# jkxing/EPSM_Mitsuba3

Hardware: AMD Instinct MI355X
Metric: manifold_paths_per_s (higher is better)
Workload: dtype f32

## Files before the change

### __graft_entry__.py

```python
from __future__ import annotations

import os
import subprocess
import sys

ROOT = os.path.dirname(os.path.abspath(__file__))
if ROOT not in sys.path:
    sys.path.insert(0, ROOT)


def build() -> None:
    env = dict(os.environ)
    targets = [("epsm_mitsuba3_amd/csrc", "epsm_mitsuba3_amd/libepsm_hip.so"),
               ("oracle", "oracle/libepsm_oracle.so"),
               ("examples", "examples/build/epsm_host_driver"),
               ("tests/host_harness", "tests/host_harness/libtrace_host.so")]
    for d, out in targets:
        path = os.path.join(ROOT, out)
        before = os.path.getmtime(path) if os.path.isfile(path) else None
        subprocess.run(["make", "-C", os.path.join(ROOT, d), "-s"], check=True, env=env)
        after = os.path.getmtime(path)
        print(f"build_mode {out}: {'up-to-date' if before == after else 'compiled'}", flush=True)
    for script, out in (("_forward_host.py", "tests/host_harness/libtrace_fwd_host.so"),
                        ("_texture_host.py", "tests/host_harness/libtrace_tex_host.so"),
                        ("_bsdf_host.py", "tests/host_harness/libtrace_bsdf_host.so"),
                        ("_material_host.py", "tests/host_harness/libtrace_material_host.so"),
                        ("_alphamap_host.py", "tests/host_harness/libtrace_alphamap_host.so")):
        path = os.path.join(ROOT, out)
        before = os.path.getmtime(path) if os.path.isfile(path) else None
        subprocess.run([sys.executable, "-B", os.path.join(ROOT, "tests", script)], check=True,
                       env=dict(env, PYTHONPATH=ROOT + os.pathsep + env.get("PYTHONPATH", "")))
        after = os.path.getmtime(path) if os.path.isfile(path) else None
        print(f"build_mode {out}: {'up-to-date' if before == after else 'compiled'}", flush=True)
    import epsm_mitsuba3_amd
    from epsm_mitsuba3_amd import _lib
    lib = _lib.lib()
    assert lib.epsm_abi_version() == _lib.ABI_VERSION == 7


def smoke() -> None:
    import torch
    import epsm_mitsuba3_amd as epsm
    from epsm_mitsuba3_amd.synth import synth_path_info, path_info_to
    from oracle.binding import oracle_calc_grad

    assert torch.cuda.is_available(), "smoke() needs cuda:0"
# ... 58 lines not shown
```

### epsm_mitsuba3_amd/_lib.py

```python
from __future__ import annotations

import ctypes as C
import os
import subprocess

import torch

_HERE = os.path.dirname(os.path.abspath(__file__))
ABI_VERSION = 7
LIB_PATH = os.path.join(_HERE, os.environ.get("EPSM_LIB_NAME", "libepsm_hip.so"))
_lib = None


class EpsmError(RuntimeError):
    pass


class build_lock:

    def __init__(self, directory: str):
        self.path = os.path.join(directory, ".build.lock")

    @staticmethod
    def _open(path: str):
# ... 202 lines not shown
    global _lib
    if _lib is None:
        if not os.path.isfile(LIB_PATH):
            raise EpsmError(
                f"{LIB_PATH} not found: build it with `python -c 'import __graft_entry__ as g; g.build()'` "
                "(or make -C epsm_mitsuba3_amd/csrc). There is no CPU fallback.")
        _lib = _declare(C.CDLL(LIB_PATH))
        if _lib.epsm_abi_version() != ABI_VERSION:
            raise EpsmError("libepsm_hip.so ABI version mismatch")
    return _lib


def stream(device):
    device = torch.device(device)
    return torch.cuda.current_stream(device).cuda_stream if device.type == "cuda" else None


def check(rc: int, what: str):
    if rc != 0:
        msg = lib().epsm_last_error().decode("utf-8", "replace")
        raise EpsmError(f"{what} failed with code {rc}: {msg}")


OPT_SMALL_WAVEFRONT_PATHS, OPT_REPLICAS, OPT_ONE_LAUNCH = 0, 1, 2


class options:

    def __init__(self, small_wavefront_paths=None, replicas=None, one_launch=None):
        self.want = {OPT_SMALL_WAVEFRONT_PATHS: small_wavefront_paths, OPT_REPLICAS: None if replicas is None else int(bool(replicas)),
                     OPT_ONE_LAUNCH: None if one_launch is None else int(bool(one_launch))}

    def __enter__(self):
        self.saved = {k: lib().epsm_get_option(k) for k, v in self.want.items() if v is not None}
        for k, v in self.want.items():
            if v is not None:
                check(lib().epsm_set_option(k, int(v)), "epsm_set_option")
        return self

    def __exit__(self, *exc):
        for k, v in self.saved.items():
            lib().epsm_set_option(k, v)
        return False
```

### epsm_mitsuba3_amd/csrc/epsm_backward_cp.hip

```cpp
#include <stdlib.h>
#include <string.h>

#define EPSM_FAST_RCP64
#include "epsm_fused.h"
#include "epsm_cp_core.h"
#include "epsm_wave_scatter.h"

using namespace epsm;

namespace {

#ifndef EPSM_CP_THREADS
#define EPSM_CP_THREADS 256
#endif
#ifndef EPSM_CP_OCC
#define EPSM_CP_OCC 3
#endif
#ifndef EPSM_CP_ROWS_FLOAT
#define EPSM_CP_ROWS_FLOAT 2064
#endif
#ifndef EPSM_CP_ROWS_FIXED
#define EPSM_CP_ROWS_FIXED 1184
#endif
#ifndef EPSM_CP_QUEUE
#define EPSM_CP_QUEUE 192
#endif
#ifndef EPSM_CP_BLOCKS
#define EPSM_CP_BLOCKS (1 << 20)
#endif
constexpr int kThreads = EPSM_CP_THREADS, kWaves = kThreads / 64, kQueueCap = EPSM_CP_QUEUE;
constexpr int kKeys = 6;
constexpr int kStashFirstItem = 64;
static_assert(kQueueCap - kStashFirstItem >= 128, "the stash needs 128 queue items");

__device__ __forceinline__ int div_small(int lane, int c) {
    const int inv = c == 1 ? 65536 : c == 2 ? 32768 : c == 3 ? 21846 : c == 4 ? 16384 : 13108;
    return (lane * inv) >> 16;
}

__device__ __forceinline__ int up1_bits(int v) { return __builtin_amdgcn_update_dpp(v, v, 0x138, 0xf, 0xf, false); }
__device__ __forceinline__ int down1_bits(int v) { return __builtin_amdgcn_update_dpp(v, v, 0x130, 0xf, 0xf, false); }
__device__ __forceinline__ float up1(float v) { return __int_as_float(up1_bits(__float_as_int(v))); }
__device__ __forceinline__ float down1(float v) { return __int_as_float(down1_bits(__float_as_int(v))); }
__device__ __forceinline__ int up1(int v) { return up1_bits(v); }
__device__ __forceinline__ int down1(int v) { return down1_bits(v); }
// ... 114 lines not shown
        }
        {
            gm = fin(gm);
            bool v = on && nz3(gm) && bid < (uint64_t) F.B;
            if (__ballot(v) != 0ull) {
                V3<float> val[1] = {mk3<float>(v ? dot(gm, dhf) : 0.f, 0.f, 0.f)};
                const uint32_t aid[3] = {2u * (uint32_t) F.V + bid, 0u, 0u};
                push<1>(v, aid, val);
            }
        }
        {
            gdiff = fin(gdiff);
            const bool v = live && nz3(gdiff) && tri_ok(tn, F.V) && (tn.w & kModePos);
            group(v, gdiff, nb0, nb1, tn.x, tn.y, tn.z);
        }
        {
            const float dis = bits_to_float(sh.w);
            const bool v = d1 && nz3(dpf) && tri_ok(ts, F.V) && (ts.w & kModePos) && dis != 0.f;
            group(v, dpf * dis, bits_to_float(sh.y), bits_to_float(sh.z), ts.x, ts.y, ts.z);
        }
    }
};

struct LaneId { int q, c, k; uint32_t plan; int loc; };
struct Rounds {
    int cls[kKeys + 1], rb[kKeys + 1];
    const uint16_t *perm;
    const uint32_t *plan;
    __device__ __forceinline__ LaneId lane_of(int r, int lane) const {
        LaneId L;
        int q = 0;
#pragma unroll
        for (int t = 1; t < kKeys; ++t) if (r >= rb[t]) q = t;
        int cls_q = cls[0], n_q = cls[1] - cls[0], rb_q = rb[0], ppr = 64;
#pragma unroll
        for (int t = 1; t < kKeys; ++t) if (q == t) { cls_q = cls[t]; n_q = cls[t + 1] - cls[t]; rb_q = rb[t]; ppr = 64 / t; }
        const int c = q > 0 ? q : 1;
        const int j = div_small(lane, c), k = lane - j * c + 1;
        const int idx = (r - rb_q) * ppr + j;
        const bool lane_on = r >= 0 && r < rb[kKeys] && j < ppr && idx < n_q;
        const int loc = lane_on ? (int) perm[cls_q + idx] : 0;
        L.q = q; L.c = c; L.k = k; L.loc = loc;
        L.plan = lane_on ? plan[loc] : 0u;
        return L;
    }
};

typedef float F2v __attribute__((ext_vector_type(2)));
typedef float F3v __attribute__((ext_vector_type(3)));
struct GeoFetch {
    F4v o0, o1, o2, o3, o4, o5;
    float o_lz;
    F4v p0, p1, p2;
    F4v n0, n1, n2;
    float gx, gy;
};
struct AddrFetch {
    F4v q6;
    F4v q7;
    U4 sh;
};
__device__ __forceinline__ F2v ld2(const float *p) { return *(const __attribute__((address_space(1))) F2v *) p; }
struct WinBase {
    const float *verts, *rays;
    const float *sub_rec;
    int64_t sub_path;
// ... 15 lines not shown
        B.sub_path = (p >= 0 && p < F.g.N) ? p : 0;
        B.sub_rec = F.pk_verts + B.sub_path * F.pk_path_stride;
    }
    B.rays = F.pk_rays + base * F.pk_ray_stride;
    B.shadow = F.pk_shadow ? F.pk_shadow + 4 * base : nullptr;
    B.list = F.pk_list ? F.pk_list + base : nullptr;
    const int64_t p0 = F.tin.path_offset + base, q0 = p0 / F.tin.spp;
    B.small = (int64_t) F.tin.res * F.tin.res < (1 << 24) && q0 + 4096 < (1 << 24) && F.tin.spp < (1 << 20);
    B.pix0 = (uint32_t) q0; B.rem0 = (uint32_t) (p0 - q0 * F.tin.spp);
    B.rcp_spp = 1.f / (float) F.tin.spp; B.rcp_res = 1.f / (float) F.tin.res;
    return B;
}
__device__ __forceinline__ void divmod24(uint32_t x, uint32_t d, float rcp_d, uint32_t &qo, uint32_t &ro) {
    uint32_t q = (uint32_t) ((float) x * rcp_d);
    int32_t r = (int32_t) x - (int32_t) (q * d);
    if (r < 0) { --q; r += (int32_t) d; }
    if (r >= (int32_t) d) { ++q; r -= (int32_t) d; }
    qo = q; ro = (uint32_t) r;
}
struct LaneRole { bool ok, first, live, end_next, d1, act1; uint32_t loc; const float *rec, *rays; const uint32_t *shadow; int64_t path; };
template <bool LIST>
__device__ __forceinline__ LaneRole role_of(const FusedArgs &F, const LaneId &L, const WinBase &B) {
    LaneRole R;
    R.ok = L.plan != 0u;
    R.first = L.k == 1;
    R.live = R.ok && L.q > 0;
    R.end_next = R.live && L.k == L.c && L.k + 1 <= cp::plan_nv(L.plan);
    R.d1 = R.ok && R.first && cp::plan_diffuse1(L.plan);
    R.act1 = (L.plan & cp::kPlanActive1) != 0;
    R.loc = R.ok ? (uint32_t) L.loc : 0u;
    if (LIST && B.list) {
        const int64_t i = R.ok ? (int64_t) lds_(B.list, (int64_t) R.loc) : B.sub_path;
        R.path = i;
        R.rec = F.pk_verts + i * F.pk_path_stride + (L.k - 1) * kRecWords;
        R.rays = F.pk_rays + i * F.pk_ray_stride;
        R.shadow = F.pk_shadow ? F.pk_shadow + 4 * i : nullptr;
        return R;
    }
    R.path = -1;
    R.rec = B.verts + (uint32_t) (R.loc * (uint32_t) F.pk_path_stride + (uint32_t) (L.k - 1) * (uint32_t) kRecWords);
    R.rays = B.rays + (uint32_t) F.pk_ray_stride * R.loc;
    R.shadow = B.shadow ? B.shadow + 4 * R.loc : nullptr;
    return R;
}
__device__ __attribute__((noinline)) int64_t pixel_offset_large(int64_t path, int spp, int res, int img_width) {
    const int64_t pix = path / spp, y = pix / res;
    return y * img_width + (pix - y * res);
}
__device__ __forceinline__ const float *pixel_grad(const TangentIn &A, const WinBase &B, uint32_t loc, int64_t path = -1) {
    if (path >= 0) return A.grad_img + pixel_offset_large(A.path_offset + path, A.spp, A.res, A.img_width) * A.img_channels + 3;
    if (!B.small) return A.grad_img + pixel_offset_large(A.path_offset + B.base + loc, A.spp, A.res, A.img_width) * A.img_channels + 3;
    int64_t y, x;
// ... 1 lines not shown
        uint32_t q1, r1, yy, xx;
        divmod24(B.rem0 + loc, (uint32_t) A.spp, B.rcp_spp, q1, r1);
        divmod24(B.pix0 + q1, (uint32_t) A.res, B.rcp_res, yy, xx);
        y = yy; x = xx;
    }
    return A.grad_img + (y * A.img_width + x) * A.img_channels + 3;
}
typedef __attribute__((address_space(3))) const F4v LdsF4;
typedef __attribute__((address_space(3))) F4v LdsF4w;
template <bool LIST>
__device__ __forceinline__ void geo_issue_rest(GeoFetch &X, const FusedArgs &F, const LaneId &L, const WinBase &B) {
    const LaneRole R = role_of<LIST>(F, L, B);
    const float *rays = R.rays;
    X.p0 = ldq(rays, 0); X.p1 = ldq(rays, 1); X.p2 = ldq(rays, 2);
    const F2v g = ld2(pixel_grad(F.tin, B, R.loc, R.path));
    X.gx = g.x; X.gy = g.y;
    const float *nx = R.end_next ? R.rec + kRecWords : B.sub_rec;
    X.n0 = ldq(nx, 0); X.n1 = ldq(nx, 1); X.n2 = ldq(nx, 2);
}
template <int VARIANT, bool LIST>
__device__ __forceinline__ void addr_issue(AddrFetch &A, const FusedArgs &F, const LaneId &L, const WinBase &B) {
    const LaneRole R = role_of<LIST>(F, L, B);
    if (R.live) {
        const bool wN = VARIANT == EPSM_VARIANT_MANIFOLD && cp::plan_a(L.plan, L.k);
        if (F.galpha || wN) A.q7 = ldq(R.rec, 7);
        if (wN) A.q6 = ldq(R.rec, 6);
    }
    if (R.d1 && R.shadow) A.sh = load_u4(R.shadow, 0);
}

template <int VARIANT, bool LIST>
__device__ __forceinline__ void own_issue(GeoFetch &X, AddrFetch &A, const FusedArgs &F, const LaneId &L, const WinBase &B) {
    const LaneRole R = role_of<LIST>(F, L, B);
    const float *rec012 = (R.live || R.d1) ? R.rec : B.sub_rec, *rec345 = R.live ? R.rec : B.sub_rec;
    X.o0 = ldq(rec012, 0); X.o1 = ldq(rec012, 1); X.o2 = ldq(rec012, 2);
    X.o3 = ldq(rec345, 3); X.o4 = ldq(rec345, 4); X.o5 = ldq(rec345, 5);
    addr_issue<VARIANT, LIST>(A, F, L, B);
}
__device__ __forceinline__ void fetch_zero(GeoFetch &X, AddrFetch &A) {
    const F4v z4 = {0.f, 0.f, 0.f, 0.f};
    A.q6 = A.q7 = z4; A.sh.x = kNoIndex; A.sh.y = A.sh.z = A.sh.w = 0u;
}

#ifndef EPSM_CP_WINDOW
#define EPSM_CP_WINDOW 2048
#endif

template <int VARIANT, int DMODE, bool PACKED, bool FLOAT_ROWS, int kWindow, bool DROP>
__global__ __launch_bounds__(kThreads, EPSM_CP_OCC) void epsm_backward_cp_kernel(FusedArgs F, int dcols, int64_t windows_per_block, int window) {
    constexpr bool kFloatRows = FLOAT_ROWS;
    constexpr int kRowsFixed = kWindow > 1024 ? EPSM_CP_ROWS_FIXED - 224 * ((kWindow - 1024) / 1024) : EPSM_CP_ROWS_FIXED;
    constexpr int kRowsFloat = kWindow > 1024 ? EPSM_CP_ROWS_FLOAT - 384 * ((kWindow - 1024) / 1024) : EPSM_CP_ROWS_FLOAT;
    typedef LdsTable<kFloatRows ? kRowsFloat : kRowsFixed, typename std::conditional<kFloatRows, AccFloat, AccFixed64>::type> Table;
    constexpr int kTableSize = Table::kTableSize;
    __shared__ uint32_t s_keys[kTableSize];
    __shared__ typename Table::Val s_vals[kTableSize * 3];
    __shared__ int s_used;
    __shared__ QItem s_queue[kWaves][kQueueCap];
    __shared__ PtrTable s_ptrs;
    float *const my_rep = F.rep ? F.rep + (blockIdx.x % (unsigned) F.replicas) * F.rep_stride : nullptr;
    const Table T{s_keys, s_vals, &s_used, my_rep ? my_rep : F.gpos, my_rep ? my_rep + 3 * F.V : F.gnrm,
                  my_rep ? my_rep + 6 * F.V : F.galpha, (uint32_t) F.V};
    const int wv = __builtin_amdgcn_readfirstlane((int) (threadIdx.x >> 6)), lane = threadIdx.x & 63;
    WaveQueue<kQueueCap> Q{s_queue[wv], 0};
    const Emitter<Table> E{F, T, Q};
    if (!PACKED && threadIdx.x < F.K) { s_ptrs.v[threadIdx.x] = F.g.v[threadIdx.x]; s_ptrs.s[threadIdx.x] = F.s[threadIdx.x]; }
    constexpr int kPer = (kWindow + kThreads - 1) / kThreads;
    constexpr int kSortKeys = DROP ? kKeys + 1 : kKeys;
    constexpr bool kList = DROP && PACKED;
    constexpr int kStride = kPer * kWaves, kEntries = kSortKeys * kStride;
    __shared__ uint32_t s_plan[kWindow];
    __shared__ uint16_t s_perm[kWindow];
    __shared__ int s_cnt[kEntries];
    __shared__ int s_cls[kKeys + 2];
    V3<float> gd_acc = zero3<float>();
    const int64_t n_slots = (kList && F.pk_list) ? (int64_t) lds_(F.pk_list_count, (int64_t) 0) : F.g.N;
    const int64_t n_windows = (n_slots + window - 1) / window;
    if (kList && !F.rep_done && (int64_t) blockIdx.x * windows_per_block >= n_windows) return;
    T.clear();
#pragma unroll 1
    for (int64_t wi = 0; wi < windows_per_block; ++wi) {
        const int64_t win = (int64_t) blockIdx.x * windows_per_block + wi;
        if (win >= n_windows) break;
        const int64_t base = win * window;
        const WinBase WB = win_base<kList>(F, base);
        int key[kPer], rank[kPer];
        {
            uint32_t fw[kPer];
#pragma unroll
            for (int j = 0; j < kPer; ++j) {
                int64_t p = base + j * kThreads + threadIdx.x;
                if (kList && F.pk_list) p = p < n_slots ? (int64_t) lds_(F.pk_list, p) : -1;
                const Records<PACKED> R{F, s_ptrs, (p >= 0 && p < F.g.N) ? p : F.g.N - 1};
                fw[j] = (j * kThreads + (int) threadIdx.x < window && p >= 0 && p < F.g.N) ? R.flag_word() : 0u;
            }
#pragma unroll
            for (int j = 0; j < kPer; ++j) {
                const int loc = j * kThreads + threadIdx.x;
                const int64_t p = base + loc;
                const bool in = loc < window && p < n_slots;
                uint32_t w = fw[j];
                if (F.K < 5) w &= (1u << (5 * F.K)) - 1u;
                uint32_t plan = VARIANT == EPSM_VARIANT_MANIFOLD ? cp::manifold_plan(w) : cp::caustic_plan(w);
                plan = in ? (plan | cp::kPlanInRange | ((w & 4u) ? cp::kPlanActive1 : 0u)) : 0u;
                const bool none = kSortKeys > kKeys && (!in || (cp::plan_m(plan) == 0 && !cp::plan_diffuse1(plan)));
                key[j] = none ? kKeys : cp::plan_m(plan);
                if (loc < window) s_plan[loc] = plan;
            }
        }
#pragma unroll
        for (int j = 0; j < kPer; ++j) {
            const bool has = j * kThreads + (int) threadIdx.x < window;
#pragma unroll
            for (int q = 0; q < kSortKeys; ++q) {
                const unsigned long long m = __ballot(has && key[j] == q);
                if (key[j] == q) rank[j] = __builtin_amdgcn_mbcnt_hi((unsigned) (m >> 32), __builtin_amdgcn_mbcnt_lo((unsigned) m, 0u));
                if (lane == 0) s_cnt[(q * kPer + j) * kWaves + wv] = __popcll(m);
            }
        }
        __syncthreads();
        if (wv == 0) {
            int carry = 0;
#pragma unroll
            for (int q0 = 0; q0 < kEntries; q0 += 64) {
                const int q = q0 + lane;
                const int c = q < kEntries ? s_cnt[q] : 0;
                int inc = c;
#pragma unroll
                for (int off = 1; off < 64; off <<= 1) { const int t = __shfl_up(inc, off); if (lane >= off) inc += t; }
                if (q < kEntries) {
                    s_cnt[q] = carry + inc - c;
                    if (q % kStride == 0) s_cls[q / kStride] = carry + inc - c;
                }
                carry += __shfl(inc, 63);
            }
            if (lane == 0) s_cls[kSortKeys] = window;
        }
        __syncthreads();
#pragma unroll
        for (int j = 0; j < kPer; ++j) {
            const int loc = j * kThreads + threadIdx.x;
            if (loc < window) s_perm[s_cnt[(key[j] * kPer + j) * kWaves + wv] + rank[j]] = (uint16_t) loc;
        }
        __syncthreads();
        Rounds RS;
        RS.perm = s_perm; RS.plan = s_plan;
#pragma unroll
        for (int q = 0; q <= kKeys; ++q) RS.cls[q] = __builtin_amdgcn_readfirstlane(s_cls[q]);
        RS.rb[0] = 0;
#pragma unroll
        for (int q = 0; q < kKeys; ++q) {
            const int c = q > 0 ? q : 1, ppr = 64 / c;
            RS.rb[q + 1] = RS.rb[q] + (RS.cls[q + 1] - RS.cls[q] + ppr - 1) / ppr;
        }
        const int n_rounds = RS.rb[kKeys];
        LaneId L = RS.lane_of(wv, lane);
        GeoFetch Xp; AddrFetch Ap;
        fetch_zero(Xp, Ap);
        if (PACKED) own_issue<VARIANT, kList>(Xp, Ap, F, L, WB);
#pragma unroll 1
        for (int r = wv; r < n_rounds; r += kWaves) {
            const int q = L.q, c = L.c, k = L.k;
            const uint32_t plan = L.plan;
            const bool ok = plan != 0u, first = k == 1;
            const int64_t i = base + L.loc;
            const Records<PACKED> R{F, s_ptrs, i};
            const int nv = cp::plan_nv(plan);
            const bool live = ok && q > 0;
            const bool has_next = live && k + 1 <= nv;
            const bool d1 = ok && first && cp::plan_diffuse1(plan);
            const bool act1 = (plan & cp::kPlanActive1) != 0;

            asm volatile("; EPSM_MARK round_begin");
            cp::Own<float> own;
            if (!PACKED) {
                own.x = own.e1 = own.e2 = own.n = own.dn1 = own.dn2 = own.light = zero3<float>();
                own.b0 = own.b1 = own.eta = 0.f;
            }
            cp::Nbr<float> prev, next;
            prev.x = prev.e1 = prev.e2 = next.x = next.e1 = next.e2 = zero3<float>();
            V2<float> dk = mk2<float>(0.f, 0.f);
            V3<float> dp = zero3<float>();
            const bool wN = VARIANT == EPSM_VARIANT_MANIFOLD && live && cp::plan_a(plan, k);
            float nb0 = 0.f, nb1 = 0.f;
            uint32_t tid_own = kNoIndex, tid_next = kNoIndex, bid = kNoIndex, etri = kNoIndex;
            V3<float> dhf = zero3<float>();
            float eb0 = 0.f, eb1 = 0.f, ew = 0.f;
            U4 sh; sh.x = kNoIndex; sh.y = sh.z = sh.w = 0u;
            if (PACKED) {
                GeoFetch X;
                geo_issue_rest<kList>(X, F, L, WB);
                X.o0 = Xp.o0; X.o1 = Xp.o1; X.o2 = Xp.o2; X.o3 = Xp.o3; X.o4 = Xp.o4; X.o5 = Xp.o5;
                Q.drain_full_groups(T);
                {
// ... 240 lines not shown
            if (threadIdx.x == 0) F.rep_done[rix] = 0u;
        }
    }
}

template <int VARIANT, int DMODE, bool PACKED>
hipError_t launch(const FusedArgs &F0, int dcols, hipStream_t s) {
    FusedArgs F = F0;
    const bool small = F.g.N <= fused_option(EPSM_OPT_SMALL_WAVEFRONT_PATHS);
#ifndef EPSM_CP_SLOTS
#define EPSM_CP_SLOTS 768
#endif
#ifndef EPSM_CP_WINDOW_CAUSTIC
#define EPSM_CP_WINDOW_CAUSTIC 2048
#endif
    constexpr int kSmall = 1024, kSlots = EPSM_CP_SLOTS;
    constexpr int kLargeRT = VARIANT == EPSM_VARIANT_MANIFOLD ? EPSM_CP_WINDOW : EPSM_CP_WINDOW_CAUSTIC;
    constexpr int kLarge = kLargeRT > 1024 ? EPSM_CP_WINDOW : 1024;
    int window = kLargeRT;
    if (small) {
        const int64_t w = ((F.g.N + kSlots - 1) / kSlots + 63) / 64 * 64;
        window = (int) (w < 128 ? 128 : w > kSmall ? kSmall : w);
    }
    const int64_t windows = (F.g.N + window - 1) / window;
    const int64_t blocks = windows < EPSM_CP_BLOCKS ? windows : EPSM_CP_BLOCKS;
    const int64_t per = (windows + blocks - 1) / blocks;
    F.rep = nullptr; F.replicas = 1; F.rep_stride = 0; F.rep_done = nullptr; F.rep_blocks = 0;
    if (small) {
        const int64_t stride = (6 * F.V + F.B + 3 + 63) / 64 * 64;
        int64_t R = blocks / 16;
        if (R > 32) R = 32;
        if (R * stride * 4 > (int64_t) kReplicaBudget) R = (int64_t) kReplicaBudget / (stride * 4);
        if (R >= 4 && fused_option(EPSM_OPT_REPLICAS) != 0) {
            const hipError_t e = fused_workspace(s, (size_t) (R * stride * 4), &F.rep);
            if (e != hipSuccess) return e;
            if (F.rep) {
                F.replicas = (int) R; F.rep_stride = stride;
                F.rep_blocks = (int) blocks;
                F.rep_done = fused_option(EPSM_OPT_ONE_LAUNCH) != 0 ? (uint32_t *) ((char *) F.rep + kReplicaBudget) : nullptr;
            }
        }
    }
    const bool float_rows = !(F.g.clip <= 1.f);
    const bool drop = DMODE != kTangentsInKernel || F.grad_o_sum == nullptr;
#define EPSM_CP_LAUNCH(FLOAT_ROWS_, WINDOW_, DROP_) \
    hipLaunchKernelGGL((epsm_backward_cp_kernel<VARIANT, DMODE, PACKED, FLOAT_ROWS_, WINDOW_, (DROP_) || DMODE != kTangentsInKernel>), \
                       dim3((unsigned) blocks), dim3(kThreads), 0, s, F, dcols, per, window)
    if (float_rows) {
        if (small) { if (drop) EPSM_CP_LAUNCH(true, kSmall, true); else EPSM_CP_LAUNCH(true, kSmall, false); }
        else { if (drop) EPSM_CP_LAUNCH(true, kLarge, true); else EPSM_CP_LAUNCH(true, kLarge, false); }
    } else {
        if (small) { if (drop) EPSM_CP_LAUNCH(false, kSmall, true); else EPSM_CP_LAUNCH(false, kSmall, false); }
        else { if (drop) EPSM_CP_LAUNCH(false, kLarge, true); else EPSM_CP_LAUNCH(false, kLarge, false); }
    }
#undef EPSM_CP_LAUNCH
    hipError_t le = hipGetLastError();
    if (le == hipSuccess && F.rep && !F.rep_done) {
        const int64_t n = 6 * F.V + F.B + 3;
        hipLaunchKernelGGL(reduce_replicas_kernel, dim3((unsigned) ((n + 255) / 256)), dim3(256), 0, s, F.rep, F.replicas, F.rep_stride,
                           F.V, F.B, F.gpos, F.gnrm, F.galpha, F.grad_o_sum);
        le = hipGetLastError();
    }
    if (le != hipSuccess && F.rep) fused_workspace_invalidate(s);
    return le;
}
template <int VARIANT, bool PACKED> hipError_t launch_d(int dmode, const FusedArgs &F, int dcols, hipStream_t s) {
    switch (dmode) {
        case kTangentsTwoColumns: return launch<VARIANT, kTangentsTwoColumns, PACKED>(F, dcols, s);
        case kTangentsFullRows: return launch<VARIANT, kTangentsFullRows, PACKED>(F, dcols, s);
        default: return launch<VARIANT, kTangentsInKernel, PACKED>(F, dcols, s);
// ... 18 lines not shown
```

### epsm_mitsuba3_amd/csrc/epsm_cp_core.h

```cpp
#pragma once

#include "epsm_path_core.h"

namespace epsm {
namespace cp {

constexpr uint32_t kPlanInRange = 1u << 20, kPlanActive1 = 1u << 21;
EPSM_HD int plan_nv(uint32_t p) { return (int) ((p >> 10) & 7u); }
EPSM_HD int plan_m(uint32_t p) { return (int) ((p >> 16) & 7u); }
EPSM_HD int plan_idstar(uint32_t p) { return (int) ((p >> 13) & 7u); }
EPSM_HD bool plan_a(uint32_t p, int k) { return ((p >> (k - 1)) & 1u) != 0; }
EPSM_HD bool plan_b(uint32_t p, int k) { return ((p >> (4 + k)) & 1u) != 0; }
EPSM_HD bool plan_diffuse1(uint32_t p) { return ((p >> 19) & 1u) != 0; }

EPSM_HD bool fbit(uint32_t w, int k, uint32_t bit) { return k >= 1 && k <= 5 && ((w >> (5 * (k - 1))) & bit) != 0; }

EPSM_HD uint32_t manifold_plan(uint32_t w) {
    bool valid = true;
    int hasdiffuse = 0, nv = 0;
    bool nvN = false;
    uint32_t a = 0, b = 0;
#pragma unroll
    for (int id = 1; id <= 5; ++id) {
        valid = valid && fbit(w, id, 16u);
        hasdiffuse += fbit(w, id, 1u) ? 1 : 0;
        valid = valid && (hasdiffuse < 2);
        const bool spec = valid && (hasdiffuse == 0);
        const bool wN = spec && fbit(w, id, 4u) && fbit(w, id, 8u);
        const bool wC = spec && fbit(w, id + 1, 4u) && fbit(w, id + 1, 1u);
        if (wN) { nv = id; nvN = true; a |= 1u << (id - 1); }
        if (wC) { nv = id + 1; nvN = false; b |= 1u << (id - 1); }
    }
    const int m = nvN ? nv : (nv > 0 ? nv - 1 : 0);
    return a | (b << 5) | ((uint32_t) nv << 10) | (nvN ? 1u << 13 : 0u) | ((uint32_t) m << 16) | (fbit(w, 1, 1u) ? 1u << 19 : 0u);
}
EPSM_HD uint32_t caustic_plan(uint32_t w) {
// ... 299 lines not shown
```

### epsm_mitsuba3_amd/csrc/epsm_grad_scatter.hip

```cpp
#include <stdlib.h>
#include <atomic>
#include <mutex>
#include <stdio.h>
#include <string.h>

#include "epsm_fused.h"

using namespace epsm;
using epsm_host::fail;

namespace epsm {

__global__ __launch_bounds__(256) void reduce_replicas_kernel(float *rep, int replicas, int64_t stride, int64_t V, int64_t B,
                                                              float *gpos, float *gnrm, float *galpha, float *go) {
    const int64_t e = (int64_t) blockIdx.x * 256 + threadIdx.x, n = 6 * V + B + 3;
    if (e >= n) return;
    float sum = 0.f;
#pragma unroll 8
    for (int r = 0; r < replicas; ++r) sum += __builtin_nontemporal_load(rep + r * stride + e);
    for (int r = 0; r < replicas; ++r) rep[r * stride + e] = 0.f;
    float *dst = e < 3 * V ? gpos + e : e < 6 * V ? gnrm + (e - 3 * V) : e < 6 * V + B ? (galpha ? galpha + (e - 6 * V) : nullptr)
                                                                                      : (go ? go + (e - 6 * V - B) : nullptr);
    if (dst && sum != 0.f && fabsf(sum) < __builtin_inff()) atomicAdd(dst, sum);
}
// ... 74 lines not shown
            !v.bsdf || !v.active || !v.active_em || !v.ismesh || !s.tri)
            return bad("NULL pointer in a vertex / scatter record");
        if (((((uintptr_t) s.aux) | ((uintptr_t) s.emit) | ((uintptr_t) s.shadow)) & 15) || (((uintptr_t) s.tri) & 3))
            return bad("aux/emit/shadow must be 16-byte aligned (tri: 4)");
        VertexPtrs<float> &o = F.g.v[k];
        o.p0 = (const float *) v.p0; o.p1 = (const float *) v.p1; o.p2 = (const float *) v.p2;
        o.n0 = (const float *) v.n0; o.n1 = (const float *) v.n1; o.n2 = (const float *) v.n2;
        o.b0 = (const float *) v.b0; o.b1 = (const float *) v.b1; o.eta = (const float *) v.eta;
        o.light = (const float *) v.light;
        o.bsdf = v.bsdf; o.active = v.active; o.active_em = v.active_em; o.ismesh = v.ismesh;
        ScatterPtrs<float> &t = F.s[k];
        t.tri = s.tri; t.aux = s.aux; t.emit = s.emit;
        t.shadow = k == 0 ? s.shadow : nullptr;
    }
    F.g.clip = (clip > 0.0f && clip <= 3.402823466e+38f) ? clip : 3.402823466e+38f;
    F.gpos = grad_pos; F.gnrm = grad_nrm; F.galpha = grad_alpha;
    F.V = V; F.B = grad_alpha ? B : 0;
    F.P = epsm_num_param_grads(variant, K);
    F.K = K;
    return EPSM_OK;
}

namespace {
std::atomic<int64_t> g_options[3];
struct OptionsInit {
    OptionsInit() {
        const char *e = getenv("EPSM_SMALL_WAVEFRONT");
        g_options[EPSM_OPT_SMALL_WAVEFRONT_PATHS] = e ? atoll(e) : (int64_t) 1 << 20;
        const char *off = getenv("EPSM_NO_REPLICAS");
        g_options[EPSM_OPT_REPLICAS] = (off && off[0] == '1') ? 0 : 1;
        const char *one = getenv("EPSM_ONE_LAUNCH");
        g_options[EPSM_OPT_ONE_LAUNCH] = (one && one[0] == '1') ? 1 : 0;
    }
} g_options_init;
}
namespace epsm {
int64_t fused_option(int option) { return g_options[option].load(std::memory_order_relaxed); }
}
extern "C" int epsm_set_option(int option, int64_t value) {
    epsm_host::err_buf()[0] = 0;
    if (option < 0 || option > EPSM_OPT_ONE_LAUNCH || value < 0) return fail(EPSM_EINVAL, "epsm_set_option: unknown option or negative value");
    g_options[option].store(value, std::memory_order_relaxed);
    return EPSM_OK;
}
extern "C" int64_t epsm_get_option(int option) {
    return (option < 0 || option > EPSM_OPT_ONE_LAUNCH) ? -1 : g_options[option].load(std::memory_order_relaxed);
}

extern "C" int epsm_release_workspace(void) {
    epsm_host::err_buf()[0] = 0;
    const hipError_t e = fused_release_workspaces();
    if (e != hipSuccess) return epsm_host::hip_fail("epsm_release_workspace", e);
    return EPSM_OK;
}

extern "C" int epsm_manifold_grad_scatter(int variant, int64_t N, int K,
                                          const float *cam, const EpsmVertexRecord *verts,
                                          const EpsmScatterRecord *sc, const uint32_t *tri_table, int64_t T,
                                          const float *dlduv, int64_t dlduv_stride, int dlduv_cols,
                                          const float *dldp, float clip,
                                          float *grad_pos, float *grad_nrm, float *grad_alpha,
                                          int64_t V, int64_t B, void *stream) {
    epsm_host::err_buf()[0] = 0;
    if (N == 0 && K >= 1 && K <= EPSM_MAX_VERTICES &&
        (variant == EPSM_VARIANT_MANIFOLD || variant == EPSM_VARIANT_MANIFOLD_CAUSTIC)) return EPSM_OK;
    FusedArgs F;
    const int rc = fill_args(F, "epsm_manifold_grad_scatter", variant, N, K, cam, verts, sc, tri_table, T, clip, grad_pos, grad_nrm, grad_alpha, V, B);
    if (rc != EPSM_OK) return rc;
    if (!dlduv || !dldp) return fail(EPSM_EINVAL, "epsm_manifold_grad_scatter: NULL argument");
// ... 82 lines not shown
```

### epsm_mitsuba3_amd/csrc/epsm_wave_scatter.h

```cpp
#pragma once

#include <hip/hip_runtime.h>
#include "epsm_path_core.h"

namespace epsm {

struct Runs {
    int head;
    bool tail;
};

__device__ __forceinline__ int lane_id() { return __lane_id(); }

__device__ __forceinline__ Runs make_runs(bool valid, uint32_t k0, uint32_t k1, uint32_t k2) {
    const int lane = lane_id();
    const uint32_t p0 = __shfl_up(k0, 1), p1 = __shfl_up(k1, 1), p2 = __shfl_up(k2, 1);
    const int pv = __shfl_up((int) valid, 1);
    const bool head = (lane == 0) || !pv || !valid || p0 != k0 || p1 != k1 || p2 != k2;
    const unsigned long long heads = __ballot(head);
    const unsigned long long below = (lane == 63) ? ~0ull : ((2ull << lane) - 1ull);
    Runs r;
    r.head = 63 - __clzll((long long) (heads & below));
    r.tail = valid && ((lane == 63) || ((heads >> (lane + 1)) & 1ull));
    return r;
// ... 9 lines not shown
    return v;
}
__device__ __forceinline__ V3<float> seg_sum3(V3<float> v, int head) {
    return mk3<float>(seg_sum(v.x, head), seg_sum(v.y, head), seg_sum(v.z, head));
}

constexpr uint32_t kEmptyKey = 0xFFFFFFFFu;
#ifndef EPSM_MAX_PROBE
#define EPSM_MAX_PROBE 4
#endif
constexpr int kMaxProbe = EPSM_MAX_PROBE;

struct AccFloat {
    typedef float T;
    static constexpr bool kBucketed = false;
    __device__ __forceinline__ static bool fits(float, float, float) { return true; }
    __device__ __forceinline__ static void add(T *p, float x) { if (fabsf(x) < __builtin_inff()) atomicAdd(p, x); }
    __device__ __forceinline__ static float get(T q) { return q; }
};
__device__ __forceinline__ bool adds_something(float x) { return x != 0.f && fabsf(x) < __builtin_inff(); }
struct AccFixed64 {
    typedef long long T;
    static constexpr bool kBucketed = true;
    static constexpr float kLimit = 16.f;
    __device__ __forceinline__ static bool fits(float x, float y, float z) {
        return fabsf(x) < kLimit && fabsf(y) < kLimit && fabsf(z) < kLimit;
    }
    __device__ __forceinline__ static T to_fixed(float x) {
        const double y = __builtin_fma((double) x, 17592186044416.0, 6755399441055744.0);
        return __double_as_longlong(y) - 0x4338000000000000LL;
    }
    __device__ __forceinline__ static void add(T *p, float x) { atomicAdd((unsigned long long *) p, (unsigned long long) to_fixed(x)); }
    __device__ __forceinline__ static float get(T q) { return (float) ((double) q * 5.6843418860808015e-14); }
};

template <int kRows, typename Acc = AccFloat>
struct LdsTable {
    static constexpr int kTableSize = kRows;
    typedef typename Acc::T Val;
    uint32_t *keys;
    Val *vals;
    int *used;
    float *gpos, *gnrm, *galpha;
    uint32_t V;

    __device__ __forceinline__ void global_add(uint32_t key, float x, float y, float z) const {
        float *p;
// ... 244 lines not shown
```

### include/epsm.h

```cpp
#ifndef EPSM_H
#define EPSM_H

#include <stddef.h>
#include <stdint.h>

#ifdef __cplusplus
extern "C" {
#endif

#define EPSM_ABI_VERSION 7

#define EPSM_BSDF_NULL     0x1u
#define EPSM_BSDF_DIFFUSE  0x6u

#define EPSM_MAX_VERTICES 5

enum {
    EPSM_VARIANT_MANIFOLD = 0,
    EPSM_VARIANT_MANIFOLD_CAUSTIC = 1
};

enum {
    EPSM_OK = 0,
    EPSM_EINVAL = -22,
// ... 73 lines not shown
    const void *verts;
    const uint32_t *shadow;
    int64_t ray_stride, path_stride;
    const uint32_t *path_list;
    const uint32_t *path_count;
} EpsmPackedLog;
#define EPSM_FLAG_DIFFUSE   1u
#define EPSM_FLAG_NULL      2u
#define EPSM_FLAG_ACTIVE    4u
#define EPSM_FLAG_ACTIVE_EM 8u
#define EPSM_FLAG_ISMESH    16u

int epsm_backward_pass_packed(int variant, int64_t N, int K, int64_t path_offset, int spp, int res,
                              const EpsmPackedLog *log, const float *grad_img, int img_width, int img_channels,
                              const uint32_t *tri_table, int64_t T, float clip,
                              float *grad_pos, float *grad_nrm, float *grad_alpha, float *grad_o_sum,
                              int64_t V, int64_t B, void *stream);

int epsm_release_workspace(void);

#define EPSM_OPT_SMALL_WAVEFRONT_PATHS 0
#define EPSM_OPT_REPLICAS 1
#define EPSM_OPT_ONE_LAUNCH 2
int epsm_set_option(int option, int64_t value);
int64_t epsm_get_option(int option);

int epsm_sinkhorn_splits(int64_t n, int64_t m);
size_t epsm_sinkhorn_scratch_bytes(int64_t n, int64_t m, int D);
int epsm_sinkhorn_softmin(int64_t n, int64_t m, int D, const float *x, const float *y, const float *h, float eps,
                          float *out, float *wsum, void *scratch, size_t scratch_bytes, void *stream);
int epsm_sinkhorn_update(int64_t n, int64_t m, int D, const float *x, const float *y, const float *dual, float log_weight,
                         float eps, const float *prev, float *out, float *wsum, void *scratch, size_t scratch_bytes, void *stream);

const char *epsm_last_error(void);

int epsm_abi_version(void);

#ifdef __cplusplus
}
#endif
#endif
```

Measured before the change: 9.756 billion.

## Pack per-path plan and slot index into one LDS word; add tail-window schedule

Merges the separate s_plan and s_perm shared arrays into a single packed 32-bit slot word that holds plan bits and the slot index. This cuts LDS footprint and removes one indirect lookup per lane, and the freed space goes to more table rows. It also adds an optional schedule that splits tail windows into half and quarter sizes to balance load, controlled by a new workgroup-slots option that defaults to 0 (off). Sort ranks are now stored in the packed register word instead of separate arrays.

New measurement: 10.07 billion, median of 6. 3.3% higher.

```diff
diff --git a/__graft_entry__.py b/__graft_entry__.py
--- a/__graft_entry__.py
+++ b/__graft_entry__.py
@@ -21,7 +21,8 @@
         subprocess.run(["make", "-C", os.path.join(ROOT, d), "-s"], check=True, env=env)
         after = os.path.getmtime(path)
         print(f"build_mode {out}: {'up-to-date' if before == after else 'compiled'}", flush=True)
-    for script, out in (("_forward_host.py", "tests/host_harness/libtrace_fwd_host.so"),
+    for script, out in (("_window_host.py", "tests/host_harness/libcp_window_host.so"),
+                        ("_forward_host.py", "tests/host_harness/libtrace_fwd_host.so"),
                         ("_texture_host.py", "tests/host_harness/libtrace_tex_host.so"),
                         ("_bsdf_host.py", "tests/host_harness/libtrace_bsdf_host.so"),
                         ("_material_host.py", "tests/host_harness/libtrace_material_host.so"),
diff --git a/epsm_mitsuba3_amd/_lib.py b/epsm_mitsuba3_amd/_lib.py
--- a/epsm_mitsuba3_amd/_lib.py
+++ b/epsm_mitsuba3_amd/_lib.py
@@ -248,14 +248,14 @@
         raise EpsmError(f"{what} failed with code {rc}: {msg}")
 
 
-OPT_SMALL_WAVEFRONT_PATHS, OPT_REPLICAS, OPT_ONE_LAUNCH = 0, 1, 2
+OPT_SMALL_WAVEFRONT_PATHS, OPT_REPLICAS, OPT_ONE_LAUNCH, OPT_WORKGROUP_SLOTS = 0, 1, 2, 3
 
 
 class options:
 
-    def __init__(self, small_wavefront_paths=None, replicas=None, one_launch=None):
+    def __init__(self, small_wavefront_paths=None, replicas=None, one_launch=None, workgroup_slots=None):
         self.want = {OPT_SMALL_WAVEFRONT_PATHS: small_wavefront_paths, OPT_REPLICAS: None if replicas is None else int(bool(replicas)),
-                     OPT_ONE_LAUNCH: None if one_launch is None else int(bool(one_launch))}
+                     OPT_ONE_LAUNCH: None if one_launch is None else int(bool(one_launch)), OPT_WORKGROUP_SLOTS: workgroup_slots}
 
     def __enter__(self):
         self.saved = {k: lib().epsm_get_option(k) for k, v in self.want.items() if v is not None}
diff --git a/epsm_mitsuba3_amd/csrc/epsm_backward_cp.hip b/epsm_mitsuba3_amd/csrc/epsm_backward_cp.hip
--- a/epsm_mitsuba3_amd/csrc/epsm_backward_cp.hip
+++ b/epsm_mitsuba3_amd/csrc/epsm_backward_cp.hip
@@ -17,10 +17,10 @@
 #define EPSM_CP_OCC 3
 #endif
 #ifndef EPSM_CP_ROWS_FLOAT
-#define EPSM_CP_ROWS_FLOAT 2064
+#define EPSM_CP_ROWS_FLOAT 2192
 #endif
 #ifndef EPSM_CP_ROWS_FIXED
-#define EPSM_CP_ROWS_FIXED 1184
+#define EPSM_CP_ROWS_FIXED 1256
 #endif
 #ifndef EPSM_CP_QUEUE
 #define EPSM_CP_QUEUE 192
@@ -181,11 +181,10 @@
     }
 };
 
-struct LaneId { int q, c, k; uint32_t plan; int loc; };
+struct LaneId { int q, c, k; uint32_t word; int loc; };
 struct Rounds {
     int cls[kKeys + 1], rb[kKeys + 1];
-    const uint16_t *perm;
-    const uint32_t *plan;
+    const uint32_t *slot;
     __device__ __forceinline__ LaneId lane_of(int r, int lane) const {
         LaneId L;
         int q = 0;
@@ -198,9 +197,8 @@
         const int j = div_small(lane, c), k = lane - j * c + 1;
         const int idx = (r - rb_q) * ppr + j;
         const bool lane_on = r >= 0 && r < rb[kKeys] && j < ppr && idx < n_q;
-        const int loc = lane_on ? (int) perm[cls_q + idx] : 0;
-        L.q = q; L.c = c; L.k = k; L.loc = loc;
-        L.plan = lane_on ? plan[loc] : 0u;
+        const uint32_t word = lane_on ? slot[cls_q + idx] : 0u;
+        L.q = q; L.c = c; L.k = k; L.word = word; L.loc = cp::slot_of(word);
         return L;
     }
 };
@@ -262,12 +260,12 @@
 template <bool LIST>
 __device__ __forceinline__ LaneRole role_of(const FusedArgs &F, const LaneId &L, const WinBase &B) {
     LaneRole R;
-    R.ok = L.plan != 0u;
+    R.ok = L.word != 0u;
     R.first = L.k == 1;
     R.live = R.ok && L.q > 0;
-    R.end_next = R.live && L.k == L.c && L.k + 1 <= cp::plan_nv(L.plan);
-    R.d1 = R.ok && R.first && cp::plan_diffuse1(L.plan);
-    R.act1 = (L.plan & cp::kPlanActive1) != 0;
+    R.end_next = R.live && L.k == L.c && L.k + 1 <= cp::plan_nv(L.word);
+    R.d1 = R.ok && R.first && cp::slot_diffuse1(L.word);
+    R.act1 = cp::slot_active1(L.word);
     R.loc = R.ok ? (uint32_t) L.loc : 0u;
     if (LIST && B.list) {
         const int64_t i = R.ok ? (int64_t) lds_(B.list, (int64_t) R.loc) : B.sub_path;
@@ -315,7 +313,7 @@
 __device__ __forceinline__ void addr_issue(AddrFetch &A, const FusedArgs &F, const LaneId &L, const WinBase &B) {
     const LaneRole R = role_of<LIST>(F, L, B);
     if (R.live) {
-        const bool wN = VARIANT == EPSM_VARIANT_MANIFOLD && cp::plan_a(L.plan, L.k);
+        const bool wN = VARIANT == EPSM_VARIANT_MANIFOLD && cp::plan_a(L.word, L.k);
         if (F.galpha || wN) A.q7 = ldq(R.rec, 7);
         if (wN) A.q6 = ldq(R.rec, 6);
     }
@@ -339,11 +337,29 @@
 #define EPSM_CP_WINDOW 2048
 #endif
 
+struct WindowRange { int64_t first, count; };
+__device__ __forceinline__ int64_t uniform64(int64_t v) {
+    const uint32_t lo = (uint32_t) __builtin_amdgcn_readfirstlane((int) (uint32_t) v), hi = (uint32_t) __builtin_amdgcn_readfirstlane((int) (uint32_t) ((uint64_t) v >> 32));
+    return (int64_t) (((uint64_t) hi << 32) | lo);
+}
+__device__ __attribute__((noinline)) WindowRange launch_windows(int64_t n, int slots, int bulk_window, int64_t workgroups) {
+    const cp::WindowSchedule s = cp::window_schedule(n, (int64_t) slots, bulk_window);
+    return WindowRange{s.windows, cp::windows_per_workgroup(s.windows, workgroups)};
+}
+__device__ __attribute__((noinline)) WindowRange window_range(int64_t n, int slots, int bulk_window, int64_t win) {
+    int64_t first;
+    int size;
+    cp::window_at(cp::window_schedule(n, (int64_t) slots, bulk_window), win, first, size);
+    return WindowRange{first, (int64_t) size};
+}
+
 template <int VARIANT, int DMODE, bool PACKED, bool FLOAT_ROWS, int kWindow, bool DROP>
-__global__ __launch_bounds__(kThreads, EPSM_CP_OCC) void epsm_backward_cp_kernel(FusedArgs F, int dcols, int64_t windows_per_block, int window) {
+__global__ __launch_bounds__(kThreads, EPSM_CP_OCC) void epsm_backward_cp_kernel(FusedArgs F, int dcols, int slots, int bulk_window) {
     constexpr bool kFloatRows = FLOAT_ROWS;
-    constexpr int kRowsFixed = kWindow > 1024 ? EPSM_CP_ROWS_FIXED - 224 * ((kWindow - 1024) / 1024) : EPSM_CP_ROWS_FIXED;
-    constexpr int kRowsFloat = kWindow > 1024 ? EPSM_CP_ROWS_FLOAT - 384 * ((kWindow - 1024) / 1024) : EPSM_CP_ROWS_FLOAT;
+    constexpr int kRowsFixed = kWindow > 1024 ? EPSM_CP_ROWS_FIXED - 152 * ((kWindow - 1024) / 1024) : EPSM_CP_ROWS_FIXED;
+    constexpr int kRowsFloat = kWindow > 1024 ? EPSM_CP_ROWS_FLOAT - 256 * ((kWindow - 1024) / 1024) : EPSM_CP_ROWS_FLOAT;
+    static_assert(kWindow % 256 == 0 && kWindow <= 4096 && kWindow <= cp::kMaxWindowSlots, "a slot below 4096 (WinBase::small), quarter windows on multiples of 64");
+    static_assert(kFloatRows || (double) kWindow * 16.0 * (double) AccFixed64::kLimit <= 524288.0, "AccFixed64: a window's terms may wrap a row");
     typedef LdsTable<kFloatRows ? kRowsFloat : kRowsFixed, typename std::conditional<kFloatRows, AccFloat, AccFixed64>::type> Table;
     constexpr int kTableSize = Table::kTableSize;
     __shared__ uint32_t s_keys[kTableSize];
@@ -362,22 +378,26 @@
     constexpr int kSortKeys = DROP ? kKeys + 1 : kKeys;
     constexpr bool kList = DROP && PACKED;
     constexpr int kStride = kPer * kWaves, kEntries = kSortKeys * kStride;
-    __shared__ uint32_t s_plan[kWindow];
-    __shared__ uint16_t s_perm[kWindow];
+    __shared__ uint32_t s_slot[kWindow];
     __shared__ int s_cnt[kEntries];
     __shared__ int s_cls[kKeys + 2];
     V3<float> gd_acc = zero3<float>();
-    const int64_t n_slots = (kList && F.pk_list) ? (int64_t) lds_(F.pk_list_count, (int64_t) 0) : F.g.N;
-    const int64_t n_windows = (n_slots + window - 1) / window;
+    int64_t n_slots = F.g.N;
+    if (kList && F.pk_list) { const int64_t cnt = (int64_t) lds_(F.pk_list_count, (int64_t) 0); n_slots = cnt < F.g.N ? cnt : F.g.N; }
+    const WindowRange WL = launch_windows(n_slots, slots, bulk_window, (int64_t) gridDim.x);
+    const int64_t n_windows = uniform64(WL.first), windows_per_block = uniform64(WL.count);
     if (kList && !F.rep_done && (int64_t) blockIdx.x * windows_per_block >= n_windows) return;
     T.clear();
 #pragma unroll 1
     for (int64_t wi = 0; wi < windows_per_block; ++wi) {
         const int64_t win = (int64_t) blockIdx.x * windows_per_block + wi;
         if (win >= n_windows) break;
-        const int64_t base = win * window;
+        const WindowRange WR = window_range(n_slots, slots, bulk_window, win);
+        const int64_t base = uniform64(WR.first);
+        const int window = __builtin_amdgcn_readfirstlane((int) WR.count);
         const WinBase WB = win_base<kList>(F, base);
-        int key[kPer], rank[kPer];
+        constexpr int kRankShift = 22;
+        uint32_t pw[kPer];
         {
             uint32_t fw[kPer];
 #pragma unroll
@@ -397,8 +417,7 @@
                 uint32_t plan = VARIANT == EPSM_VARIANT_MANIFOLD ? cp::manifold_plan(w) : cp::caustic_plan(w);
                 plan = in ? (plan | cp::kPlanInRange | ((w & 4u) ? cp::kPlanActive1 : 0u)) : 0u;
                 const bool none = kSortKeys > kKeys && (!in || (cp::plan_m(plan) == 0 && !cp::plan_diffuse1(plan)));
-                key[j] = none ? kKeys : cp::plan_m(plan);
-                if (loc < window) s_plan[loc] = plan;
+                pw[j] = (plan & ~(7u << 16)) | ((none ? (uint32_t) kKeys : (uint32_t) cp::plan_m(plan)) << 16);
             }
         }
 #pragma unroll
@@ -406,8 +425,9 @@
             const bool has = j * kThreads + (int) threadIdx.x < window;
 #pragma unroll
             for (int q = 0; q < kSortKeys; ++q) {
-                const unsigned long long m = __ballot(has && key[j] == q);
-                if (key[j] == q) rank[j] = __builtin_amdgcn_mbcnt_hi((unsigned) (m >> 32), __builtin_amdgcn_mbcnt_lo((unsigned) m, 0u));
+                const bool mine = cp::plan_m(pw[j]) == q;
+                const unsigned long long m = __ballot(has && mine);
+                if (mine) pw[j] |= __builtin_amdgcn_mbcnt_hi((unsigned) (m >> 32), __builtin_amdgcn_mbcnt_lo((unsigned) m, 0u)) << kRankShift;
                 if (lane == 0) s_cnt[(q * kPer + j) * kWaves + wv] = __popcll(m);
             }
         }
@@ -433,11 +453,12 @@
 #pragma unroll
         for (int j = 0; j < kPer; ++j) {
             const int loc = j * kThreads + threadIdx.x;
-            if (loc < window) s_perm[s_cnt[(key[j] * kPer + j) * kWaves + wv] + rank[j]] = (uint16_t) loc;
+            const int key = cp::plan_m(pw[j]), rank = (int) ((pw[j] >> kRankShift) & 63u);
+            if (loc < window) s_slot[s_cnt[(key * kPer + j) * kWaves + wv] + rank] = cp::slot_word(pw[j], (uint32_t) loc);
         }
         __syncthreads();
         Rounds RS;
-        RS.perm = s_perm; RS.plan = s_plan;
+        RS.slot = s_slot;
 #pragma unroll
         for (int q = 0; q <= kKeys; ++q) RS.cls[q] = __builtin_amdgcn_readfirstlane(s_cls[q]);
         RS.rb[0] = 0;
@@ -454,15 +475,15 @@
 #pragma unroll 1
         for (int r = wv; r < n_rounds; r += kWaves) {
             const int q = L.q, c = L.c, k = L.k;
-            const uint32_t plan = L.plan;
+            const uint32_t plan = L.word;
             const bool ok = plan != 0u, first = k == 1;
             const int64_t i = base + L.loc;
             const Records<PACKED> R{F, s_ptrs, i};
             const int nv = cp::plan_nv(plan);
             const bool live = ok && q > 0;
             const bool has_next = live && k + 1 <= nv;
-            const bool d1 = ok && first && cp::plan_diffuse1(plan);
-            const bool act1 = (plan & cp::kPlanActive1) != 0;
+            const bool d1 = ok && first && cp::slot_diffuse1(plan);
+            const bool act1 = cp::slot_active1(plan);
 
             asm volatile("; EPSM_MARK round_begin");
             cp::Own<float> own;
@@ -749,9 +770,10 @@
         const int64_t w = ((F.g.N + kSlots - 1) / kSlots + 63) / 64 * 64;
         window = (int) (w < 128 ? 128 : w > kSmall ? kSmall : w);
     }
-    const int64_t windows = (F.g.N + window - 1) / window;
+    const int64_t opt_slots = fused_option(EPSM_OPT_WORKGROUP_SLOTS);
+    const int slots = small ? 0 : (int) (opt_slots < (1 << 20) ? opt_slots : (1 << 20));
+    const int64_t windows = cp::window_schedule(F.g.N, slots, window).windows;
     const int64_t blocks = windows < EPSM_CP_BLOCKS ? windows : EPSM_CP_BLOCKS;
-    const int64_t per = (windows + blocks - 1) / blocks;
     F.rep = nullptr; F.replicas = 1; F.rep_stride = 0; F.rep_done = nullptr; F.rep_blocks = 0;
     if (small) {
         const int64_t stride = (6 * F.V + F.B + 3 + 63) / 64 * 64;
@@ -772,7 +794,7 @@
     const bool drop = DMODE != kTangentsInKernel || F.grad_o_sum == nullptr;
 #define EPSM_CP_LAUNCH(FLOAT_ROWS_, WINDOW_, DROP_) \
     hipLaunchKernelGGL((epsm_backward_cp_kernel<VARIANT, DMODE, PACKED, FLOAT_ROWS_, WINDOW_, (DROP_) || DMODE != kTangentsInKernel>), \
-                       dim3((unsigned) blocks), dim3(kThreads), 0, s, F, dcols, per, window)
+                       dim3((unsigned) blocks), dim3(kThreads), 0, s, F, dcols, slots, window)
     if (float_rows) {
         if (small) { if (drop) EPSM_CP_LAUNCH(true, kSmall, true); else EPSM_CP_LAUNCH(true, kSmall, false); }
         else { if (drop) EPSM_CP_LAUNCH(true, kLarge, true); else EPSM_CP_LAUNCH(true, kLarge, false); }
diff --git a/epsm_mitsuba3_amd/csrc/epsm_cp_core.h b/epsm_mitsuba3_amd/csrc/epsm_cp_core.h
--- a/epsm_mitsuba3_amd/csrc/epsm_cp_core.h
+++ b/epsm_mitsuba3_amd/csrc/epsm_cp_core.h
@@ -12,6 +12,52 @@
 EPSM_HD bool plan_a(uint32_t p, int k) { return ((p >> (k - 1)) & 1u) != 0; }
 EPSM_HD bool plan_b(uint32_t p, int k) { return ((p >> (4 + k)) & 1u) != 0; }
 EPSM_HD bool plan_diffuse1(uint32_t p) { return ((p >> 19) & 1u) != 0; }
+
+constexpr int kSlotShift = 19, kMaxWindowSlots = 1 << (32 - kSlotShift);
+EPSM_HD uint32_t slot_word(uint32_t plan, uint32_t slot) {
+    if (!(plan & kPlanInRange)) return 0u;
+    return (plan & 0xffffu) | (((plan >> 19) & 1u) << 16) | (((plan >> 21) & 1u) << 17) | (1u << 18) | (slot << kSlotShift);
+}
+EPSM_HD bool slot_diffuse1(uint32_t s) { return ((s >> 16) & 1u) != 0; }
+EPSM_HD bool slot_active1(uint32_t s) { return ((s >> 17) & 1u) != 0; }
+EPSM_HD bool slot_in_range(uint32_t s) { return ((s >> 18) & 1u) != 0; }
+EPSM_HD int slot_of(uint32_t s) { return (int) (s >> kSlotShift); }
+
+struct WindowSchedule {
+    int64_t n;
+    int64_t start_half, start_quarter;
+    int64_t win_half, win_quarter;
+    int64_t windows;
+    int w_bulk, w_half, w_quarter;
+};
+EPSM_HD WindowSchedule window_schedule(int64_t n, int64_t S, int W) {
+    WindowSchedule s;
+    s.n = n < 0 ? 0 : n;
+    s.w_bulk = W; s.w_half = S > 0 ? W / 2 : W; s.w_quarter = S > 0 ? W / 4 : W;
+    s.start_half = s.start_quarter = 0;
+    if (S > 0) {
+        const int64_t cap_q = S * (int64_t) (W / 4), cap_h = S * (int64_t) (W / 2);
+        const int64_t tail_q = s.n < cap_q ? s.n : cap_q;
+        s.start_quarter = (s.n - tail_q) / W * W;
+        const int64_t tail_h = s.start_quarter < cap_h ? s.start_quarter : cap_h;
+        s.start_half = (s.start_quarter - tail_h) / W * W;
+    }
+    s.win_half = s.start_half / s.w_bulk;
+    s.win_quarter = s.win_half + (s.start_quarter - s.start_half) / s.w_half;
+    s.windows = s.win_quarter + (s.n - s.start_quarter + s.w_quarter - 1) / s.w_quarter;
+    return s;
+}
+EPSM_HD void window_at(const WindowSchedule &s, int64_t win, int64_t &first, int &size) {
+    int w;
+    if (win < s.win_half) { first = win * s.w_bulk; w = s.w_bulk; }
+    else if (win < s.win_quarter) { first = s.start_half + (win - s.win_half) * s.w_half; w = s.w_half; }
+    else { first = s.start_quarter + (win - s.win_quarter) * s.w_quarter; w = s.w_quarter; }
+    const int64_t left = s.n - first;
+    size = left < (int64_t) w ? (int) left : w;
+}
+EPSM_HD int64_t windows_per_workgroup(int64_t windows, int64_t workgroups) {
+    return windows <= workgroups ? 1 : (windows + workgroups - 1) / workgroups;
+}
 
 EPSM_HD bool fbit(uint32_t w, int k, uint32_t bit) { return k >= 1 && k <= 5 && ((w >> (5 * (k - 1))) & bit) != 0; }
 
diff --git a/epsm_mitsuba3_amd/csrc/epsm_grad_scatter.hip b/epsm_mitsuba3_amd/csrc/epsm_grad_scatter.hip
--- a/epsm_mitsuba3_amd/csrc/epsm_grad_scatter.hip
+++ b/epsm_mitsuba3_amd/csrc/epsm_grad_scatter.hip
@@ -120,7 +120,7 @@
 }
 
 namespace {
-std::atomic<int64_t> g_options[3];
+std::atomic<int64_t> g_options[EPSM_OPT_WORKGROUP_SLOTS + 1];
 struct OptionsInit {
     OptionsInit() {
         const char *e = getenv("EPSM_SMALL_WAVEFRONT");
@@ -129,6 +129,9 @@
         g_options[EPSM_OPT_REPLICAS] = (off && off[0] == '1') ? 0 : 1;
         const char *one = getenv("EPSM_ONE_LAUNCH");
         g_options[EPSM_OPT_ONE_LAUNCH] = (one && one[0] == '1') ? 1 : 0;
+        const char *ws = getenv("EPSM_WORKGROUP_SLOTS");
+        const int64_t wsv = ws ? atoll(ws) : 0;
+        g_options[EPSM_OPT_WORKGROUP_SLOTS] = wsv > 0 ? wsv : 0;
     }
 } g_options_init;
 }
@@ -137,12 +140,12 @@
 }
 extern "C" int epsm_set_option(int option, int64_t value) {
     epsm_host::err_buf()[0] = 0;
-    if (option < 0 || option > EPSM_OPT_ONE_LAUNCH || value < 0) return fail(EPSM_EINVAL, "epsm_set_option: unknown option or negative value");
+    if (option < 0 || option > EPSM_OPT_WORKGROUP_SLOTS || value < 0) return fail(EPSM_EINVAL, "epsm_set_option: unknown option or negative value");
     g_options[option].store(value, std::memory_order_relaxed);
     return EPSM_OK;
 }
 extern "C" int64_t epsm_get_option(int option) {
-    return (option < 0 || option > EPSM_OPT_ONE_LAUNCH) ? -1 : g_options[option].load(std::memory_order_relaxed);
+    return (option < 0 || option > EPSM_OPT_WORKGROUP_SLOTS) ? -1 : g_options[option].load(std::memory_order_relaxed);
 }
 
 extern "C" int epsm_release_workspace(void) {
diff --git a/epsm_mitsuba3_amd/csrc/epsm_wave_scatter.h b/epsm_mitsuba3_amd/csrc/epsm_wave_scatter.h
--- a/epsm_mitsuba3_amd/csrc/epsm_wave_scatter.h
+++ b/epsm_mitsuba3_amd/csrc/epsm_wave_scatter.h
@@ -55,7 +55,10 @@
 struct AccFixed64 {
     typedef long long T;
     static constexpr bool kBucketed = true;
-    static constexpr float kLimit = 16.f;
+#ifndef EPSM_FIXED_LIMIT
+#define EPSM_FIXED_LIMIT 16
+#endif
+    static constexpr float kLimit = (float) EPSM_FIXED_LIMIT;
     __device__ __forceinline__ static bool fits(float x, float y, float z) {
         return fabsf(x) < kLimit && fabsf(y) < kLimit && fabsf(z) < kLimit;
     }
diff --git a/include/epsm.h b/include/epsm.h
--- a/include/epsm.h
+++ b/include/epsm.h
@@ -119,6 +119,7 @@
 #define EPSM_OPT_SMALL_WAVEFRONT_PATHS 0
 #define EPSM_OPT_REPLICAS 1
 #define EPSM_OPT_ONE_LAUNCH 2
+#define EPSM_OPT_WORKGROUP_SLOTS 3
 int epsm_set_option(int option, int64_t value);
 int64_t epsm_get_option(int option);
 
```
